# omarezz46/BayesDLL

Hardware: AMD Instinct MI355X
Metric: SG-HMC leapfrog steps/sec & HBM GB/s on ViT-L/32 params, 1/2/4/8 MI355X (higher is better)
Workload: dtype f32

## Files before the change

bayesdll_amd/_lib.py:

```python
from __future__ import annotations

import ctypes as C
import os
import threading

import torch

HERE = os.path.dirname(os.path.abspath(__file__))
LIB_PATH = os.environ.get("BDL_SGMCMC_LIB", os.path.join(HERE, "libbdl_sgmcmc.so"))

BDL_OK = 0
CSGHMC, SGHMC, SGLD, SGHMC_GRAD, SGLD_GRAD, ADAM_SGHMC, ADAM_SGHMC_GRAD = range(7)
NOISE_NONE, NOISE_BUFFER, NOISE_PHILOX = 0, 1, 2
COLLECT_NONE, COLLECT_WELFORD_INIT, COLLECT_WELFORD, COLLECT_MEAN_INIT, COLLECT_MEAN = range(5)
MIX_BARE, MIX_PIPELINED, MIX_PACED = 0, 1, 2
ATTR_HEAD, ATTR_PRIOR, ATTR_SKIP, ATTR_GUNALIGNED = 0x1, 0x2, 0x4, 0x8
FLAG_FIRST_STEP, FLAG_RECIP_DIV, FLAG_MOMENTUM, FLAG_GRAD_READY = 0x1, 0x2, 0x4, 0x8
VAR_GIVEN, VAR_RAW_MOMENTS, VAR_WELFORD = 0, 1, 2
ABI_VERSION = 8

_fp = C.c_void_p


class Segment(C.Structure):
# ... 229 lines not shown
LOWP_UNROLLS = (1, 2, 4)

LOWP_EXPORTS = {
    "bdl_lowp_step": (C.c_int, [C.POINTER(LowpArgs), C.c_void_p]),
    "bdl_lowp_shadow": (C.c_int, [C.c_void_p, C.c_void_p, C.c_void_p, C.c_int32, C.c_int64,
                                  C.c_void_p]),
}


class LayerSegment(C.Structure):
    _fields_ = [("offset", C.c_int64), ("numel", C.c_int64)]


class DiagLayersArgs(C.Structure):
    _fields_ = [("mom1", _fp), ("mom2", _fp), ("segments", _fp), ("table", _fp),
                ("workspace", _fp), ("n", C.c_int64), ("chain_groups", C.c_uint64),
                ("nsegments", C.c_int32), ("chains", C.c_int32), ("var_mode", C.c_int32),
                ("grid_blocks", C.c_int32), ("ratio", C.c_float), ("inv_ratio", C.c_float),
                ("var_floor", C.c_float), ("c1", C.c_float), ("thresholds", C.c_float * 3),
                ("pad0", C.c_int32)]


class EssLayersArgs(C.Structure):
    _fields_ = [("sM2", _fp), ("bM2", _fp), ("segments", _fp), ("table", _fp),
                ("workspace", _fp), ("n", C.c_int64), ("chain_groups", C.c_uint64),
                ("samples", C.c_int64), ("batches", C.c_int64), ("nsegments", C.c_int32),
                ("chains", C.c_int32), ("grid_blocks", C.c_int32), ("thresholds", C.c_float * 3)]


LAYERS_MAX_SEGMENTS, LAYERS_MAX_GRID = 65536, 1024

LAYERS_EXPORTS = {
    "bdl_layers_workspace_bytes": (C.c_int64, [C.c_int32, C.c_int32]),
    "bdl_chain_diag_layers": (C.c_int, [C.POINTER(DiagLayersArgs), C.c_void_p]),
    "bdl_chain_ess_layers": (C.c_int, [C.POINTER(EssLayersArgs), C.c_void_p]),
}

PREDICT_MAX_CLASSES, PREDICT_WAVE_CLASSES, PREDICT_MAX_BINS = 8192, 256, 64
PREDICT_MAX_GROUPS, PREDICT_MAX_GRID = 65535, 1024
PREDICT_RESET = 0x1


class PredictTotals(C.Structure):
    _fields_ = [("n", C.c_int64), ("n_labelled", C.c_int64), ("n_nonfinite", C.c_int64),
                ("n_wrong", C.c_int64), ("disagree_sum", C.c_int64), ("nll_sum", C.c_double),
                ("entropy_sum", C.c_double), ("expected_entropy_sum", C.c_double),
                ("mi_sum", C.c_double), ("mi_sum_wrong", C.c_double),
                ("bin_count", C.c_int64 * PREDICT_MAX_BINS),
                ("bin_hits", C.c_int64 * PREDICT_MAX_BINS),
                ("bin_conf", C.c_double * PREDICT_MAX_BINS)]


class PredictArgs(C.Structure):
    _fields_ = [("logits", _fp), ("labels", _fp), ("logp", _fp), ("entropy", _fp),
                ("expected_entropy", _fp), ("mutual_info", _fp), ("confidence", _fp),
                ("nll", _fp), ("pred", _fp), ("disagree", _fp), ("totals", _fp),
                ("workspace", _fp), ("batch", C.c_int64), ("members", C.c_int32),
                ("groups", C.c_int32), ("classes", C.c_int32), ("num_bins", C.c_int32),
                ("grid_blocks", C.c_int32), ("flags", C.c_int32),
                ("edges", C.c_float * PREDICT_MAX_BINS)]


PREDICT_EXPORTS = {
    "bdl_predict_workspace_bytes": (C.c_int64, [C.c_int32, C.c_int32]),
    "bdl_predict": (C.c_int, [C.POINTER(PredictArgs), C.c_void_p]),
}


class FnFoldArgs(C.Structure):
    _fields_ = [("logits", _fp), ("bsum", _fp), ("smean", _fp), ("sM2", _fp), ("bM2", _fp),
                ("probs", _fp), ("probe", C.c_int64), ("chain_groups", C.c_uint64),
                ("sample", C.c_int64), ("batch", C.c_int64), ("chains", C.c_int32),
                ("classes", C.c_int32), ("flags", C.c_int32), ("fs", C.c_float),
                ("fb", C.c_float), ("c", C.c_float), ("grid_blocks", C.c_int32),
                ("pad0", C.c_int32)]


FN_MAX_CLASSES, FN_WAVE_CLASSES, FN_MAX_GRID = 8192, 256, 2048

FN_EXPORTS = {
    "bdl_fn_fold": (C.c_int, [C.POINTER(FnFoldArgs), C.c_void_p]),
}

_lib = None
_lock = threading.Lock()


def lib():
    global _lib
    if _lib is not None:
        return _lib
    with _lock:
        if _lib is None:
            if not os.path.exists(LIB_PATH):
                raise RuntimeError(
                    f"bayesdll_amd: HIP library not found at {LIB_PATH}; build it with "
                    "`make -C bayesdll_amd/csrc` (or __graft_entry__.build()). There is no CPU "
                    "fallback for the fused SG-MCMC step.")
            h = C.CDLL(LIB_PATH)
            for name, (res, argt) in (list(EXPORTS.items()) + list(DIAG_EXPORTS.items())
                                      + list(CLIP_EXPORTS.items())
                                      + list(CHAIN_STEP_EXPORTS.items())
                                      + list(STATS_EXPORTS.items())
                                      + list(ESS_EXPORTS.items())
                                      + list(LOWP_EXPORTS.items())
                                      + list(LAYERS_EXPORTS.items())
                                      + list(PREDICT_EXPORTS.items())
                                      + list(FN_EXPORTS.items())):
                fn = getattr(h, name)
                fn.restype = res
                fn.argtypes = argt
            if h.bdl_version() != ABI_VERSION:
                raise RuntimeError(f"bayesdll_amd: ABI version mismatch ({h.bdl_version()} != "
                                   f"{ABI_VERSION}); rebuild the library")
            _lib = h
    return _lib


def check(rc: int, what: str):
    if rc != BDL_OK:
        msg = lib().bdl_last_error().decode(errors="replace")
        raise RuntimeError(f"{what} failed (status {rc}): {msg}")
    return rc


def ptr(t):
    return None if t is None else C.c_void_p(t.data_ptr())


def current_stream_handle(device=None):
    return C.c_void_p(torch.cuda.current_stream(device).cuda_stream)


def require_hip(t: torch.Tensor, what: str):
    if not t.is_cuda:
        raise RuntimeError(f"bayesdll_amd: {what} must live on a HIP device (got {t.device}); "
                           "the fused SG-MCMC step has no CPU path")
    if t.dtype != torch.float32:
        raise RuntimeError(f"bayesdll_amd: {what} must be float32 (got {t.dtype})")
```

bayesdll_amd/csrc/bdl_api.hip:

```cpp
#include <algorithm>
#include "bdl_chain_common.hpp"
#include "bdl_measure.h"

#include <mutex>
#include <vector>

namespace bdl {
namespace {

thread_local std::string g_last_error;

int g_blocks_per_cu = 2;
int g_unroll = 1;
int g_grid_stride = 1;

int device_cu_count() {
  static int cached[64] = {0};
  int dev = 0;
  if (hipGetDevice(&dev) != hipSuccess || dev < 0 || dev >= 64) return 256;
  if (cached[dev] == 0) {
    int cus = 0;
    if (hipDeviceGetAttribute(&cus, hipDeviceAttributeMultiprocessorCount, dev) != hipSuccess ||
        cus <= 0)
      cus = 256;
    cached[dev] = cus;
  }
  return cached[dev];
}

constexpr int kMaxNormPartials = 2048;

template <int NOISE, bool RECIP, bool PRIOR>
__device__ __forceinline__ double sqnorm_fast(const KArgs& a, const StepConst& c, int64_t gb,
                                              float ns, double acc, const float* gp) {
  constexpr int U = 2;
  f4v th[U], g[U], t0[U], ep[U];
  const f4v z = {0.f, 0.f, 0.f, 0.f};
#pragma unroll
  for (int u = 0; u < U; ++u) {
    const int64_t e = (gb + (int64_t)u * kBlock + threadIdx.x) * 4;
    t0[u] = ep[u] = z;
    th[u] = vload(a.theta + e);
    g[u] = vload(gp + e);
    if constexpr (PRIOR) t0[u] = vload(a.prior_mean + e);
    if constexpr (NOISE == BDL_NOISE_BUFFER) ep[u] = vload(a.noise + e);
  }
#pragma unroll
  for (int u = 0; u < U; ++u) {
    const int64_t gi = gb + (int64_t)u * kBlock + threadIdx.x;
    if constexpr (NOISE == BDL_NOISE_PHILOX) ep[u] = step_noise4(a, gi);
#pragma unroll
    for (int j = 0; j < 4; ++j) {
      float xt = th[u][j], xg = g[u][j], xv = 0.f;
      update_core<BDL_SGLD_GRAD, NOISE, RECIP, PRIOR, false>(a, c, 0.f, ns, xt, xg, xv, t0[u][j],
                                                             ep[u][j]);
      acc = fma((double)xg, (double)xg, acc);
    }
  }
  return acc;
}

template <int NOISE, bool RECIP>
__device__ __forceinline__ void sqnorm_body(const KArgs& a, double* __restrict__ partials) {
  __shared__ double s_wave[kBlock / 64];
  constexpr int64_t kIter = (int64_t)kBlock * 2;
  StepConst c;
  c.sgd_mom = c.sgd_mom_read = c.has_m2 = c.grad_ready = c.clip = false;
  c.inv_s2 = a.inv_s2;
  c.inv_nd = a.inv_nd;
  c.inv_ca = c.inv_cb = c.clip_coef = 1.0f;
  const int64_t ngroups = (a.n + 3) >> 2, nfull = a.n >> 2;
  stage_runs(a);
  double acc = 0.0;
  int r = find_run_lds(a.nruns, (int64_t)blockIdx.x * kIter * 4);
  for (int64_t gb = (int64_t)blockIdx.x * kIter; gb < ngroups; gb += (int64_t)gridDim.x * kIter) {
    while (r < a.nruns - 1 && run_end(r) <= gb * 4) ++r;
    const int64_t gend = min(gb + kIter, ngroups);
    const uint32_t attr = run_attr(r);
    if (gend == gb + kIter && gend <= nfull && run_end(r) >= gend * 4 && !(attr & kNoFastPath)) {
      const float ns = (attr & BDL_ATTR_HEAD) ? a.ns1 : a.ns0;
      if (attr & BDL_ATTR_PRIOR)
        acc = sqnorm_fast<NOISE, RECIP, true>(a, c, gb, ns, acc, run_grad(a, r));
      else
        acc = sqnorm_fast<NOISE, RECIP, false>(a, c, gb, ns, acc, run_grad(a, r));
    } else {
// ... 654 lines not shown
      !p.kernelParams[0]) {
    (void)hipGetLastError();
    return fail(BDL_ERR_ARG, "bdl_graph_node_step_args: not a kernel node with arguments");
  }
  {
    std::lock_guard<std::mutex> lk(g_captured_mu);
    if (std::find(g_captured_funcs.begin(), g_captured_funcs.end(), (const void*)p.func) ==
        g_captured_funcs.end())
      return fail(BDL_ERR_ARG, "bdl_graph_node_step_args: the node runs no captured step kernel");
  }
  const KArgs* ka = (const KArgs*)p.kernelParams[0];
  const int64_t v[10] = {(int64_t)(uintptr_t)ka->theta, (int64_t)(uintptr_t)ka->grad,
                         (int64_t)(uintptr_t)ka->mom,   (int64_t)(uintptr_t)ka->runs,
                         (int64_t)(uintptr_t)ka->gbase, (int64_t)ka->nruns,
                         ka->n,                          (int64_t)ka->flags,
                         (int64_t)(uintptr_t)ka->mom1,  (int64_t)(uintptr_t)ka->mom2};
  for (int i = 0; i < 10; ++i) out[i] = v[i];
  return BDL_OK;
}

int bdl_graph_redirect(void* graph_exec, void* node) {
  if (graph_exec && !node) return fail(BDL_ERR_NULL, "bdl_graph_redirect: null node");
  g_redirect_exec = (hipGraphExec_t)graph_exec;
  g_redirect_node = graph_exec ? (hipGraphNode_t)node : nullptr;
  return BDL_OK;
}

const char* bdl_last_error(void) { return g_last_error.c_str(); }

int bdl_set_launch_config(int32_t blocks_per_cu, int32_t unroll, int32_t grid_stride) {
  const int prev = (g_grid_stride << 24) | (g_blocks_per_cu << 8) | g_unroll;
  g_blocks_per_cu = blocks_per_cu > 0 ? blocks_per_cu : 2;
  g_unroll = (unroll == 1 || unroll == 2 || unroll == 4) ? unroll : 1;
  g_grid_stride = grid_stride > 0 ? 1 : 0;
  return prev;
}

int bdl_build_runs(const bdl_segment* segs, int32_t nseg, int64_t n, bdl_run* out, int32_t max_runs) {
  if (!out || (nseg > 0 && !segs)) return fail(BDL_ERR_NULL, "bdl_build_runs: null pointer");
  if (n < 0 || nseg < 0 || max_runs < 1) return fail(BDL_ERR_ARG, "bdl_build_runs: bad sizes");
  int nr = 0;
  int64_t pos = 0;
  auto push = [&](int64_t end, uint32_t attr) -> bool {
    if (end <= pos) return true;
    if (nr > 0 && out[nr - 1].attr == attr) {
      out[nr - 1].end = end;
    } else {
      if (nr >= max_runs) return false;
      out[nr].end = end;
      out[nr].attr = attr;
      out[nr].pad = 0;
      ++nr;
    }
    pos = end;
    return true;
  };
  for (int i = 0; i < nseg; ++i) {
    const bdl_segment& s = segs[i];
    if (s.offset < pos || s.numel < 0 || s.offset + s.numel > n)
      return fail(BDL_ERR_RUNS, "bdl_build_runs: segments overlap, are unsorted or exceed n");
    if (!push(s.offset, BDL_ATTR_SKIP)) return fail(BDL_ERR_ARG, "bdl_build_runs: too many runs");
    if (!push(s.offset + s.numel, s.attr & 0xFu))
      return fail(BDL_ERR_ARG, "bdl_build_runs: too many runs");
  }
  if (!push(n, BDL_ATTR_SKIP)) return fail(BDL_ERR_ARG, "bdl_build_runs: too many runs");
  if (nr == 0) {
    out[0].end = 0;
    out[0].attr = BDL_ATTR_SKIP;
    out[0].pad = 0;
    nr = 1;
  }
  return nr;
}

int bdl_sgmcmc_step(const bdl_step_args* s, void* stream) {
  return launch_step(s, nullptr, (hipStream_t)stream);
}

int bdl_sgmcmc_step_bare(const bdl_step_args* s, void* stream) {
  if (const int rc = no_redirect("bdl_sgmcmc_step_bare")) return rc;
  if (s && s->method != BDL_CSGHMC)
    return fail(BDL_ERR_ARG, "bdl_sgmcmc_step_bare: the bare sweep exists for cSGHMC only");
  return launch_step(s, nullptr, (hipStream_t)stream, true);
}

int64_t bdl_clip_workspace_bytes(int64_t n) {
  (void)n;
  return (int64_t)16 + (int64_t)kMaxNormPartials * (int64_t)sizeof(double);
}

int bdl_sgld_step_clipped(const bdl_step_args* s, float max_norm, void* workspace, void* stream) {
  if (const int rc = no_redirect("bdl_sgld_step_clipped")) return rc;
  if (!s) return fail(BDL_ERR_NULL, "bdl_sgld_step_clipped: null args");
  if (!workspace) return fail(BDL_ERR_NULL, "bdl_sgld_step_clipped: null workspace");
  if (misaligned(workspace, 15)) return fail(BDL_ERR_ALIGN, "bdl_sgld_step_clipped: workspace not 16-B aligned");
  if (s->method != BDL_SGLD)
    return fail(BDL_ERR_ARG, "bdl_sgld_step_clipped: only the SGLD sampler clips its gradient");
  if (s->flags & BDL_FLAG_GRAD_READY)
    return fail(BDL_ERR_ARG, "bdl_sgld_step_clipped: GRAD_READY is incompatible with clipping");
  if (!(max_norm > 0.0f)) return fail(BDL_ERR_ARG, "bdl_sgld_step_clipped: max_norm must be > 0");
  if (s->n < 0) return fail(BDL_ERR_ARG, "bdl_sgmcmc_step: n < 0");
  if (s->n == 0) return BDL_OK;
  if (s->noise_mode < BDL_NOISE_NONE || s->noise_mode > BDL_NOISE_PHILOX)
    return fail(BDL_ERR_ARG, "bdl_sgld_step_clipped: unknown noise mode");
  if (!s->theta || !s->prior_mean)
    return fail(BDL_ERR_NULL, "bdl_sgld_step_clipped: theta and prior_mean are required");
  if (const int rc = check_runs_and_grad(s, "bdl_sgld_step_clipped")) return rc;
  if (s->noise_mode == BDL_NOISE_BUFFER && !s->noise)
    return fail(BDL_ERR_NULL, "bdl_sgld_step_clipped: noise buffer is required");
  hipStream_t st = (hipStream_t)stream;
  float* ws = (float*)workspace;
  double* partials = reinterpret_cast<double*>(reinterpret_cast<char*>(workspace) + 16);

  KArgs a{};
  a.theta = s->theta;
  a.grad = s->grad;
  a.prior_mean = s->prior_mean;
  a.noise = s->noise;
  a.runs = s->runs;
  a.gbase = s->grad_base;
  a.nruns = s->nruns;
  a.flags = s->flags;
  a.n = s->n;
  a.goff = s->philox_offset;
  a.cgroups = (uint32_t)s->chain_groups;
  a.ns0 = s->noise_scale[0];
  a.ns1 = s->noise_scale[1];
  a.sigma2 = s->sigma2;
  a.n_data = s->n_data;
  a.seed = s->seed;
  a.chain = s->chain;
  a.step = s->step;
  a.inv_s2 = recip_or(s->inv_sigma2, s->sigma2);
  a.inv_nd = recip_or(s->inv_n_data, s->n_data);
  const int64_t ngroups = (s->n + 3) / 4;
  const int64_t iters = (ngroups + 2 * kBlock - 1) / (2 * kBlock);
  const int64_t cap = std::min<int64_t>((int64_t)device_cu_count() * g_blocks_per_cu, kMaxNormPartials);
  const int grid = (int)capped_grid(iters, cap);
  const size_t shmem = run_lds_bytes(s);
  switch (s->noise_mode) {
    case BDL_NOISE_NONE:
      hipLaunchKernelGGL(bdl_sqnorm_kernel<BDL_NOISE_NONE>, dim3(grid), dim3(kBlock), shmem, st, a, partials);
      break;
    case BDL_NOISE_BUFFER:
      hipLaunchKernelGGL(bdl_sqnorm_kernel<BDL_NOISE_BUFFER>, dim3(grid), dim3(kBlock), shmem, st, a, partials);
      break;
    default:
      hipLaunchKernelGGL(bdl_sqnorm_kernel<BDL_NOISE_PHILOX>, dim3(grid), dim3(kBlock), shmem, st, a, partials);
      break;
  }
  hipLaunchKernelGGL(bdl_clip_finalize_kernel, dim3(1), dim3(kBlock), 0, st, partials, grid, max_norm, ws);
  if (const int rc = launched("bdl_sgld_step_clipped")) return rc;
  return launch_step(s, ws, st);
}

int bdl_adam_step(const bdl_step_args* s, const bdl_adam_args* ad, void* stream) {
  if (const int rc = no_redirect("bdl_adam_step")) return rc;
  if (!s || !ad) return fail(BDL_ERR_NULL, "bdl_adam_step: null args");
  if (s->method != BDL_ADAM_SGHMC && s->method != BDL_ADAM_SGHMC_GRAD)
    return fail(BDL_ERR_ARG, "bdl_adam_step: method must be BDL_ADAM_SGHMC or BDL_ADAM_SGHMC_GRAD");
  if (s->noise_mode < BDL_NOISE_NONE || s->noise_mode > BDL_NOISE_PHILOX)
    return fail(BDL_ERR_ARG, "bdl_adam_step: unknown noise mode");
  if (s->collect < BDL_COLLECT_NONE || s->collect > BDL_COLLECT_MEAN)
    return fail(BDL_ERR_ARG, "bdl_adam_step: unknown collect mode");
  if (s->n < 0) return fail(BDL_ERR_ARG, "bdl_adam_step: n < 0");
  if (s->n == 0) return BDL_OK;
// ... 189 lines not shown
```

bayesdll_amd/flat.py:

```python
from __future__ import annotations

import contextlib
import ctypes as C

import numpy as np
import torch

from . import _lib as L
from .arena import default_grad_arena


def segment_attrs(names, readout_name, bias, requires_grad):
    attrs = []
    for nm, rg in zip(names, requires_grad):
        a = 0
        if readout_name is not None and readout_name in nm:
            a |= L.ATTR_HEAD
        if not ("bias" in nm and bias == "uninformative"):
            a |= L.ATTR_PRIOR
        if not rg:
            a |= L.ATTR_SKIP
        attrs.append(a)
    return attrs


def build_runs(offsets, numels, attrs, n):
    nseg = len(offsets)
    segs = (L.Segment * max(nseg, 1))()
    for i, (o, k, a) in enumerate(zip(offsets, numels, attrs)):
        segs[i].offset, segs[i].numel, segs[i].attr, segs[i].pad = int(o), int(k), int(a), 0
    cap = 2 * nseg + 2
    runs = (L.Run * cap)()
    nr = L.lib().bdl_build_runs(segs, nseg, int(n), runs, cap)
    if nr < 0:
        L.check(nr, "bdl_build_runs")
    out = torch.empty(nr, 2, dtype=torch.int64)
    for i in range(nr):
        out[i, 0] = runs[i].end
        out[i, 1] = runs[i].attr
    return out


GRAD_MODES = ("tensor", "flat")
MAX_TENSOR_RUNS = 2730
GRAD_TABLE_CACHE = 8


def default_grad_mode():
    import os
    m = os.environ.get("BDL_GRAD_MODE", "tensor")
    if m not in GRAD_MODES:
        raise ValueError(f"BDL_GRAD_MODE must be one of {GRAD_MODES}, got {m!r}")
    return m


COMPUTE_DTYPES = {None: None, "fp32": None, "float32": None, torch.float32: None,
                  "bf16": torch.bfloat16, "bfloat16": torch.bfloat16,
                  torch.bfloat16: torch.bfloat16}


def check_compute_dtype(compute_dtype):
    try:
        return COMPUTE_DTYPES[compute_dtype]
    except (KeyError, TypeError):
        raise ValueError(f"bayesdll_amd: compute_dtype must be fp32 or bf16, got "
                         f"{compute_dtype!r}") from None


def refuse_lowp_network(net, ntensors, grad_mode=None):
    if (grad_mode or default_grad_mode()) != "tensor":
        raise ValueError("bayesdll_amd: bf16 compute reads autograd's bf16 gradients in place: "
                         "the flat gradient vector (BDL_GRAD_MODE=flat) is not supported")
    if ntensors > MAX_TENSOR_RUNS:
        raise ValueError(f"bayesdll_amd: bf16 compute needs one run per tensor in the kernel's "
                         f"LDS table ({ntensors} parameter tensors > {MAX_TENSOR_RUNS}); the "
                         "flat gradient fallback is not supported")
    if default_grad_arena():
        raise ValueError("bayesdll_amd: bf16 compute does not support the gradient arena "
                         "(BDL_GRAD_ARENA=1)")
    fbuf = [nm for nm, b in net.named_buffers() if b.is_floating_point()]
    if fbuf:
        raise ValueError("bayesdll_amd: bf16 compute does not support networks with "
                         f"floating-point buffers (e.g. BatchNorm running statistics): {fbuf[:3]}")


class FlatState:

    def __init__(self, net, net0=None, *, readout_name=None, bias="informative",
                 need_prior=False, need_mom=True, need_noise=False, extra=(), grad_mode=None,
                 compute_dtype=None):
        named = list(net.named_parameters())
        if not named:
            raise ValueError("bayesdll_amd: the network has no parameters")
        self.compute_dtype = check_compute_dtype(compute_dtype)
        if self.compute_dtype is not None:
            refuse_lowp_network(net, len(named), grad_mode)
        self.names = [nm for nm, _ in named]
        self.params = [p for _, p in named]
        self.shapes = [tuple(p.shape) for p in self.params]
        self.numels = [p.numel() for p in self.params]
        self.offsets = np.concatenate([[0], np.cumsum(self.numels)[:-1]]).astype(np.int64).tolist()
        self.n = int(sum(self.numels))
        dev = self.params[0].device
        for nm, p in named:
            L.require_hip(p.data, f"parameter {nm!r}")
            if p.device != dev:
                raise RuntimeError("bayesdll_amd: all parameters must be on one device")
        self.device = dev
        self.readout_name = readout_name if readout_name is not None else getattr(
            net, "readout_name", None)
        self.bias = bias
        self.requires_grad = [p.requires_grad for p in self.params]
        self.grad_mode = grad_mode or default_grad_mode()
        if self.grad_mode not in GRAD_MODES:
            raise ValueError(f"grad_mode must be one of {GRAD_MODES}")
        if self.grad_mode == "tensor" and len(self.params) > MAX_TENSOR_RUNS:
            import warnings
            warnings.warn(f"bayesdll_amd: {len(self.params)} parameter tensors > "
                          f"{MAX_TENSOR_RUNS}: using the flat gradient vector")
            self.grad_mode = "flat"

        names_ = ["theta"] + (["grad"] if self.grad_mode == "flat" else []) + \
            (["mom"] if need_mom else []) + (["prior"] if need_prior else []) + list(extra)
        vecs = {nm: torch.zeros(self.n, dtype=torch.float32, device=dev) for nm in names_}
        self.extra = {nm: vecs[nm] for nm in extra}
        self.theta = vecs["theta"]
        with torch.no_grad():
            for p, o, k in zip(self.params, self.offsets, self.numels):
                self.theta[o:o + k].copy_(p.data.reshape(-1))
                p.data = self.theta[o:o + k].view(p.shape)
        self.shadow = None
        if self.compute_dtype is not None:
            self.shadow = torch.empty(self.n, dtype=self.compute_dtype, device=dev)
            self.refresh_shadow()
            for p, o, k in zip(self.params, self.offsets, self.numels):
                p.data = self.shadow[o:o + k].view(p.shape)
        self.grad = vecs["grad"].zero_() if self.grad_mode == "flat" else None
        self.gbase = None
        self._bind_grads()
        self.arena = None
        if self.grad_mode == "tensor" and default_grad_arena():
            from .arena import GradArena
            self.arena = GradArena(dev, 4 * self.n)

        self.mom = vecs["mom"].zero_() if need_mom else None
        self.prior = None
        if need_prior:
            self.prior = vecs["prior"].zero_()
            if net0 is not None:
                p0 = list(net0.parameters())
                if [tuple(q.shape) for q in p0] != self.shapes:
                    raise ValueError("bayesdll_amd: net0 does not match net's parameter shapes")
                with torch.no_grad():
                    for q, o, k in zip(p0, self.offsets, self.numels):
                        self.prior[o:o + k].copy_(q.detach().reshape(-1))
        self.noise = torch.empty(self.n, dtype=torch.float32, device=dev) if need_noise else None
        self.nonfinite = torch.zeros(1, dtype=torch.int32, device=dev)

        attrs = segment_attrs(self.names, self.readout_name, bias, self.requires_grad)
        self.attrs = attrs
        self.runs = build_runs(self.offsets, self.numels, attrs, self.n).to(dev)
        self.nruns = int(self.runs.shape[0])
        self._base_runs = (self.runs, self.nruns)
        self._skip_tables = {}
        self._grad_tables = {}
        self._untouched = ()
        self._touched = [False] * len(self.params) if self.grad_mode == "flat" else []
        self._hooks = [p.register_post_accumulate_grad_hook(self._mark(i))
                       for i, p in enumerate(self.params) if p.requires_grad] \
            if self.grad_mode == "flat" else []

    def _mark(self, i):
        touched = self._touched

        def hook(_p):
            touched[i] = True
        return hook

    @classmethod
    def from_segments(cls, segments, readout_name, *, bias="informative", device="cuda",
                      need_prior=False, need_mom=True, need_noise=False, init=None, extra=()):
        self = cls.__new__(cls)
        self.names = [nm for nm, _ in segments]
        self.shapes = [tuple(s) for _, s in segments]
        self.numels = [int(np.prod(s)) for s in self.shapes]
        self.offsets = np.concatenate([[0], np.cumsum(self.numels)[:-1]]).astype(np.int64).tolist()
        self.n = int(sum(self.numels))
        self.device = torch.device(device)
        if self.device.type == "cuda" and self.device.index is None:
            self.device = torch.device("cuda", torch.cuda.current_device())
        self.readout_name = readout_name
        self.bias = bias
        self.requires_grad = [True] * len(self.names)
        self.params = []
        self._grad_ptrs = []
        f32 = dict(dtype=torch.float32, device=self.device)
        names_ = (["theta"] if init is None else []) + ["grad"] + (["mom"] if need_mom else []) \
            + (["prior"] if need_prior else []) + list(extra)
        vecs = {nm: torch.zeros(self.n, **f32) for nm in names_}
        self.extra = {nm: vecs[nm] for nm in extra}
        self.theta = vecs["theta"] if init is None else init
        self.grad_mode = "flat"
        self.compute_dtype = None
        self.shadow = None
        self.gbase = None
        self.arena = None
        self._grad_tables = {}
        self._untouched = ()
        self.grad = vecs["grad"].zero_()
        self.mom = vecs["mom"].zero_() if need_mom else None
        self.prior = vecs["prior"].zero_() if need_prior else None
        self.noise = torch.empty(self.n, **f32) if need_noise else None
        self.nonfinite = torch.zeros(1, dtype=torch.int32, device=self.device)
        self.attrs = segment_attrs(self.names, readout_name, bias, self.requires_grad)
        self.runs = build_runs(self.offsets, self.numels, self.attrs, self.n).to(self.device)
        self.nruns = int(self.runs.shape[0])
        self._base_runs = (self.runs, self.nruns)
        self._skip_tables = {}
        self._touched = []
        self._hooks = []
        return self

    def _bind_grads(self):
        if self.grad_mode == "tensor":
            for p in self.params:
                p.grad = None
            self._grad_ptrs = [0 if rg else None for rg in self.requires_grad]
            return
        self._grad_ptrs = []
        for p, o, k, rg in zip(self.params, self.offsets, self.numels,
                               [p.requires_grad for p in self.params]):
            if rg:
                p.grad = self.grad[o:o + k].view(p.shape)
                self._grad_ptrs.append(p.grad.data_ptr())
            else:
                self._grad_ptrs.append(None)

    def zero_grad(self):
        if self.grad_mode == "tensor":
            for p in self.params:
                p.grad = None
            return
        self.grad.zero_()
        for i in range(len(self._touched)):
            self._touched[i] = False
        for p, ptr in zip(self.params, self._grad_ptrs):
            if ptr is not None and (p.grad is None or p.grad.data_ptr() != ptr):
                self._bind_grads()
                break

    def backward_routing(self):
        if self.arena is None:
            return contextlib.nullcontext()
        return self.arena.routing()

    def sync_grads(self):
        if self.grad_mode == "tensor":
            self._sync_tensor_grads()
            return
        rebind = False
        untouched = []
        for i, (p, o, k, ptr) in enumerate(zip(self.params, self.offsets, self.numels,
                                               self._grad_ptrs)):
            if ptr is None:
                continue
            g = p.grad
            if g is None:
                self.grad[o:o + k].zero_()
                untouched.append(i)
                rebind = True
            else:
                if g.data_ptr() != ptr:
                    self.grad[o:o + k].copy_(g.reshape(-1))
                    rebind = True
                if self._touched and not self._touched[i]:
                    untouched.append(i)
        if rebind:
            self._bind_grads()
        self._select_runs(tuple(untouched))

    def _select_runs(self, untouched):
        if not untouched:
            self.runs, self.nruns = self._base_runs
            return
        tab = self._skip_tables.get(untouched)
        if tab is None:
            attrs = list(self.attrs)
            for i in untouched:
                attrs[i] |= L.ATTR_SKIP
            runs = build_runs(self.offsets, self.numels, attrs, self.n).to(self.device)
            tab = self._skip_tables[untouched] = (runs, int(runs.shape[0]))
        self.runs, self.nruns = tab

    def use_tensor_grads(self, grads):
        if len(grads) != len(self.numels):
            raise ValueError("use_tensor_grads: one gradient (or None) per segment")
        self.grad_mode, self.grad = "tensor", None
        ptrs, untouched = [], []
# ... 204 lines not shown
```

bayesdll_amd/kernels.py:

```python
from __future__ import annotations

import ctypes as C
import os

import numpy as np
import torch

from . import _lib as L
from . import ess as E

DIV_MODE = os.environ.get("BDL_DIV_MODE", "recip")


def _div_flag(div_mode=None):
    return L.FLAG_RECIP_DIV if (div_mode or DIV_MODE) == "recip" else 0


def _inv(s):
    s = float(s)
    return 1.0 / s if s != 0.0 else 0.0


def _step_args(state, method, *, lrs, noise_scale, noise_mode, one_minus_alpha=1.0,
               prior_sig=0.0, sigma2=1.0, n_data=1.0, mu=0.0, first_step=False,
# ... 119 lines not shown
        _tune_kind(state, fn, kind, written)
    _use_geometry(state, kind)
    t = getattr(state, "timer", None)
    e0 = t.begin() if t is not None else None
    fn()
    if e0 is not None:
        t.end(e0, alg_bytes_per_elem(a, adam) * int(a.n))


def _written(state, method, *, grad_only, mom, extra=(), mom1=None, mom2=None):
    if grad_only:
        if getattr(state, "grad", None) is None:
            return None
        out = [state.grad]
    else:
        out = [state.theta]
    out += [t for t in (mom,) + tuple(extra) + (mom1, mom2) if t is not None]
    return out


LOWP_UNROLL = 4


def lowp_args(state, method, *, blocks=0, unroll=LOWP_UNROLL, **kw):
    if method not in (L.CSGHMC, L.SGHMC, L.SGLD):
        raise ValueError("bayesdll_amd: compute_dtype=bf16 covers the cSGHMC, SGHMC and SGLD "
                         "steps; the *_GRAD contract (the caller steps) and Adam have no bf16 form")
    if kw.get("grad_ready"):
        raise ValueError("bayesdll_amd: the bf16 step has no GRAD_READY form (no clipped step)")
    if kw.get("mom_buf") is not None:
        raise ValueError("bayesdll_amd: the bf16 step takes its SGD buffer from state.mom")
    s = _step_args(state, method, **kw)
    a = L.LowpArgs()
    for f in ("theta", "grad", "mom", "prior_mean", "noise", "mom1", "mom2", "runs", "grad_base",
              "nonfinite", "n", "nruns", "method", "noise_mode", "collect", "flags",
              "one_minus_alpha", "prior_sig", "sigma2", "n_data", "mu", "collect_a", "collect_b",
              "inv_sigma2", "inv_n_data", "inv_collect_a", "inv_collect_b", "seed", "chain",
              "step", "philox_offset", "chain_groups"):
        setattr(a, f, getattr(s, f))
    for i in range(2):
        a.lr[i], a.noise_scale[i] = s.lr[i], s.noise_scale[i]
    a.shadow = state.shadow.data_ptr()
    a.blocks, a.unroll = int(blocks), int(unroll)
    return a


def lowp_step(state, method, **kw):
    a = lowp_args(state, method, **kw)
    t = getattr(state, "timer", None)
    e0 = t.begin() if t is not None else None
    L.check(L.lib().bdl_lowp_step(a, L.current_stream_handle(state.device)), "bdl_lowp_step")
    if e0 is not None:
        s = _step_args(state, method, **{k: v for k, v in kw.items()
                                         if k not in ("blocks", "unroll")})
        t.end(e0, alg_bytes_per_elem(s) * int(a.n))


def lowp_shadow(theta, shadow):
    if shadow.dtype != torch.bfloat16 or shadow.numel() != theta.numel():
        raise ValueError("lowp_shadow: shadow must be a bf16 tensor of theta's length")
    L.require_hip(theta, "theta")
    L.check(L.lib().bdl_lowp_shadow(theta.data_ptr(), shadow.data_ptr(), None, 0,
                                    int(theta.numel()), L.current_stream_handle(theta.device)),
            "bdl_lowp_shadow")


def sgmcmc_step(state, method, **kw):
    if getattr(state, "shadow", None) is not None:
        return lowp_step(state, method, **kw)
    a = _step_args(state, method, **kw)
    mb = kw.get("mom_buf")
    wr = _written(state, method, grad_only=method in (L.SGHMC_GRAD, L.SGLD_GRAD),
                  mom=state.mom if mb is None else mb,
                  mom1=kw.get("mom1") if kw.get("collect", L.COLLECT_NONE) else None,
                  mom2=kw.get("mom2") if kw.get("collect", L.COLLECT_NONE) else None)
    _launch(state, lambda: L.check(L.lib().bdl_sgmcmc_step(a, L.current_stream_handle(state.device)),
                                   "bdl_sgmcmc_step"), a, written=wr)


def sgmcmc_step_bare(state, **kw):
    a = _step_args(state, L.CSGHMC, **kw)
    L.check(L.lib().bdl_sgmcmc_step_bare(a, L.current_stream_handle(state.device)),
            "bdl_sgmcmc_step_bare")


def adam_step(state, method, *, adam_m, adam_v, sgd_buf=None, beta1, beta2, eps, t,
              momentum_decay, nd, temperature=1.0, grad_is_mom=False, lrs, noise_mode,
              sigma2, n_data, mu=0.0, first_step=False, momentum=False, collect=L.COLLECT_NONE,
              mom1=None, mom2=None, collect_a=1.0, collect_b=1.0, seed=0, chain=0, step=0,
              div_mode=None, noise=None, philox_offset=0):
    a = _step_args(state, method, lrs=lrs, noise_scale=(0.0, 0.0), noise_mode=noise_mode,
                   one_minus_alpha=1 - momentum_decay, sigma2=sigma2, n_data=n_data, mu=mu,
                   first_step=first_step, momentum=momentum, collect=collect, mom1=mom1,
                   mom2=mom2, collect_a=collect_a, collect_b=collect_b, seed=seed, chain=chain,
                   step=step, div_mode=div_mode, noise=noise, philox_offset=philox_offset)
    ad = L.AdamArgs()
    ad.adam_m = adam_m.data_ptr()
    ad.adam_v = adam_v.data_ptr()
    ad.sgd_buf = None if sgd_buf is None else sgd_buf.data_ptr()
    ad.beta1, ad.one_minus_beta1 = float(beta1), 1 - float(beta1)
    ad.beta2, ad.one_minus_beta2 = float(beta2), 1 - float(beta2)
    bc1, bc2 = 1 - float(beta1) ** int(t), 1 - float(beta2) ** int(t)
    ad.bias_corr1, ad.bias_corr2 = bc1, bc2
    ad.eps = float(eps)
    ad.two_alpha = 2 * float(momentum_decay)
    ad.nd = float(nd)
    ad.temperature = float(temperature)
    ad.inv_bias_corr1, ad.inv_bias_corr2 = _inv(bc1), _inv(bc2)
    ad.inv_temperature = _inv(temperature)
    ad.grad_is_mom = 1 if grad_is_mom else 0
    wr = _written(state, method, grad_only=method == L.ADAM_SGHMC_GRAD, mom=state.mom,
                  extra=(adam_m, adam_v) + ((sgd_buf,) if sgd_buf is not None else ()),
                  mom1=mom1 if collect != L.COLLECT_NONE else None,
                  mom2=mom2 if collect != L.COLLECT_NONE else None)
    _launch(state, lambda: L.check(L.lib().bdl_adam_step(a, ad, L.current_stream_handle(state.device)),
                                   "bdl_adam_step"), a, ad, written=wr)


def stream_mix(reads, writes, blocks_per_cu=1, unroll=4, schedule=L.MIX_BARE):
    n = reads[0].numel()
    dev = reads[0].device
    rp = (C.c_void_p * len(reads))(*[t.data_ptr() for t in reads])
    wp = (C.c_void_p * len(writes))(*[t.data_ptr() for t in writes])
    L.check(L.lib().bdl_stream_mix_schedule(rp, len(reads), wp, len(writes), int(n),
                                            int(blocks_per_cu), int(unroll), int(schedule),
                                            L.current_stream_handle(dev)), "bdl_stream_mix")


def clip_workspace(state):
    ws = getattr(state, "_clip_ws", None)
    if ws is None:
        nbytes = int(L.lib().bdl_clip_workspace_bytes(int(state.n)))
        ws = torch.empty((nbytes + 3) // 4, dtype=torch.float32, device=state.device)
        state._clip_ws = ws
    return ws


def sgld_step_clipped(state, max_norm, **kw):
    a = _step_args(state, L.SGLD, **kw)
    _use_geometry(state)
    ws = clip_workspace(state)
    L.check(L.lib().bdl_sgld_step_clipped(a, float(max_norm), ws.data_ptr(),
                                          L.current_stream_handle(state.device)),
            "bdl_sgld_step_clipped")
    return ws


def moments_update(theta, mom1, mom2, collect, collect_a=1.0, collect_b=1.0, div_mode=None):
    L.require_hip(theta, "theta")
    a = L.MomentsArgs()
    a.theta, a.mom1 = theta.data_ptr(), mom1.data_ptr()
    a.mom2 = None if mom2 is None else mom2.data_ptr()
    a.n = theta.numel()
    a.collect = int(collect)
    a.flags = _div_flag(div_mode)
    a.collect_a, a.collect_b = float(collect_a), float(collect_b)
    a.inv_collect_a, a.inv_collect_b = _inv(collect_a), _inv(collect_b)
    L.check(L.lib().bdl_moments_update(a, L.current_stream_handle(theta.device)),
            "bdl_moments_update")


SAMPLE_GEOMETRIES = ((1, 4), (2, 4), (3, 4), (4, 4), (4, 1), (6, 1))
SAMPLE_TUNE_MIN = 1 << 22
_SAMPLE_GEOM = {}


# ... 647 lines not shown
    a.scalars = scalars.data_ptr()
    a.n1, a.chain_groups, a.chains = int(state.n1), int(state.chain_groups), int(state.K)
    a.method, a.noise_mode, a.collect = int(method), int(noise_mode), int(collect)
    a.flags = ((L.FLAG_FIRST_STEP if first_step else 0) | (L.FLAG_MOMENTUM if momentum else 0)
               | _div_flag(div_mode))
    a.blocks_per_chain, a.unroll = int(blocks_per_chain), int(unroll)
    a.collect_a, a.collect_b = float(collect_a), float(collect_b)
    a.inv_collect_a, a.inv_collect_b = _inv(collect_a), _inv(collect_b)
    a.seed = int(seed) & 0xFFFFFFFFFFFFFFFF
    a.chain = int(chain) & 0xFFFFFFFFFFFFFFFF
    a.step = int(step) & 0xFFFFFFFFFFFFFFFF
    return a


def chain_step(state, method, *, scalars, **kw):
    K_ = int(state.K)
    if (scalars.dtype != torch.float32 or not scalars.is_cuda or not scalars.is_contiguous()
            or scalars.numel() != K_ * 12 or scalars.device != state.theta.device):
        raise ValueError("chain_step: scalars must be a contiguous float32 [K, 12] tensor on the "
                         "state's device")
    if not kw.get("blocks_per_chain"):
        kw["blocks_per_chain"] = chain_step_blocks_per_chain(state.n1, K_, state.theta.device,
                                                             kw.get("unroll") or 1)
    a = chain_step_args(state, method, scalars=scalars, **kw)
    dev = state.theta.device
    t = getattr(state, "timer", None)
    e0 = t.begin() if t is not None else None
    L.check(L.lib().bdl_chain_step(a, L.current_stream_handle(dev)), "bdl_chain_step")
    if e0 is not None:
        t.end(e0, alg_bytes_per_elem(a) * int(a.n1) * K_)


def philox_normal(n, seed, chain, step, device="cuda"):
    out = torch.empty(n, dtype=torch.float32, device=device)
    L.check(L.lib().bdl_philox_normal(out.data_ptr(), int(n), int(seed), int(chain), int(step),
                                      L.current_stream_handle(out.device)), "bdl_philox_normal")
    return out


_ACTIVE = [None]
LIBRARY_DEFAULT = (2, 1, 1)


def set_launch_config(blocks_per_cu=0, unroll=0, grid_stride=0):
    _ACTIVE[0] = (int(blocks_per_cu), int(unroll), int(grid_stride))
    return L.lib().bdl_set_launch_config(int(blocks_per_cu), int(unroll), int(grid_stride))


def restore_launch_config(packed):
    return set_launch_config((packed >> 8) & 0xFFFF, packed & 0xFF, (packed >> 24) & 0xFF)


def _use_geometry(state, kind="step"):
    cfg = getattr(state, {"collect": "collect_cfg", "init": "init_cfg"}.get(kind, "launch_cfg"),
                  None)
    if cfg is None:
        cfg = getattr(state, "launch_cfg", None)
    if cfg is not None and cfg != _ACTIVE[0]:
        set_launch_config(*cfg)


AUTOTUNE_CANDIDATES = ((2, 1, 1), (1, 4, 1), (3, 1, 1), (2, 4, 1), (1, 2, 1), (2, 2, 1))
AUTOTUNE_BY_METHOD = {
    "csghmc": AUTOTUNE_CANDIDATES + ((3, 4, 1), (1, 1, 1)),
    "sgld": AUTOTUNE_CANDIDATES + ((3, 4, 1), (4, 4, 1), (1, 1, 1)),
    "adam": AUTOTUNE_CANDIDATES + ((1, 1, 1), (4, 4, 1)),
}
_TUNED = {}
_TUNED_COLLECT = {}
COLLECT_EXTRA = ((1, 1, 1),)


ADAM_EXTRA = ("adam_m", "adam_v", "sgd_buf")


def _scratch_launcher(n, dev, method):
    return _scratch_launchers(n, dev, method)[0]


def _scratch_launchers(n, dev, method):
    from .flat import FlatState, moment_pair
    st = FlatState.from_segments([("w", (int(n),))], None, device=dev,
                                 need_prior=method != "csghmc",
                                 extra=ADAM_EXTRA if method == "adam" else ())
    st.theta.zero_()
    if method == "csghmc":
        kw = dict(lrs=(1e-4, 1e-4), noise_scale=(0.0, 0.0), noise_mode=L.NOISE_NONE,
                  one_minus_alpha=0.9, prior_sig=1.0)

        def launch():
            sgmcmc_step(st, L.CSGHMC, **kw)
    elif method == "sgld":
        st.prior.zero_()
        kw = dict(lrs=(1e-4, 1e-4), noise_scale=(1e-3, 1e-3), noise_mode=L.NOISE_PHILOX,
                  sigma2=1.0, n_data=1e6, mu=0.5, momentum=True)

        def launch():
            sgmcmc_step(st, L.SGLD, **kw)
    elif method == "adam":
        st.prior.zero_()
        m, v, buf = (st.extra[k] for k in ADAM_EXTRA)
        kw = dict(adam_m=m, adam_v=v, sgd_buf=buf, beta1=0.9, beta2=0.999, eps=1e-8, t=3,
                  momentum_decay=0.1, nd=0.01, lrs=(1e-4, 1e-4), noise_mode=L.NOISE_PHILOX,
                  sigma2=1.0, n_data=1e6, mu=0.5, momentum=True)

        def launch():
            adam_step(st, L.ADAM_SGHMC, **kw)
    else:
        raise ValueError(f"unknown method {method!r}")
    moms = []

    def launch_collect():
        if not moms:
            moms.extend(moment_pair(int(n), dev) if method == "csghmc" else
                        (torch.zeros_like(st.theta), torch.zeros_like(st.theta)))
            moms[0].copy_(st.theta)
            moms[1].zero_()
        if method == "csghmc":
            sgmcmc_step(st, L.CSGHMC, lrs=(1e-4, 1e-4), noise_scale=(1e-7, 1e-7),
                        noise_mode=L.NOISE_PHILOX, one_minus_alpha=0.9, prior_sig=1.0,
                        collect=L.COLLECT_WELFORD, mom1=moms[0], mom2=moms[1], collect_a=3.0)
        elif method == "sgld":
            sgmcmc_step(st, L.SGLD, collect=L.COLLECT_MEAN, mom1=moms[0], mom2=moms[1],
                        collect_a=2.0, collect_b=3.0, **kw)
        else:
            adam_step(st, L.ADAM_SGHMC, collect=L.COLLECT_MEAN, mom1=moms[0], mom2=moms[1],
                      collect_a=2.0, collect_b=3.0, **kw)
    return launch, launch_collect


def _device(device):
    return torch.device(device) if device is not None else torch.device(
        "cuda", torch.cuda.current_device())


def autotune(n, device=None, reps=6, candidates=None, method="csghmc", collect=False):
    import numpy as np
    dev = _device(device)
    if candidates is None:
        candidates = AUTOTUNE_BY_METHOD.get(method, AUTOTUNE_CANDIDATES)
    launch, launch_collect = _scratch_launchers(n, dev, method)

    def pick(fn, cands):
        times = measure(fn, cands, reps)
        top = sorted(times, key=times.get)[:3]
        again = measure(fn, top, 2 * reps)
        for cfg in top:
            times[cfg] = 0.5 * (times[cfg] + again[cfg])
        return min(top, key=times.get), times

    def measure(fn, cfgs, k):
        out = {}
        for cfg in cfgs:
            set_launch_config(*cfg)
            for _ in range(2):
                fn()
            ev = [(torch.cuda.Event(enable_timing=True), torch.cuda.Event(enable_timing=True))
                  for _ in range(k)]
            for e0, e1 in ev:
                e0.record()
                fn()
                e1.record()
            torch.cuda.synchronize(dev)
            out[cfg] = float(np.median([a.elapsed_time(b) for a, b in ev]))
        return out

    best, times = pick(launch, candidates)
# ... 111 lines not shown
```

Baseline: 1002.

## Pick momentum buffer placement by timing candidate allocations at construction

```diff
diff --git a/bayesdll_amd/_lib.py b/bayesdll_amd/_lib.py
--- a/bayesdll_amd/_lib.py
+++ b/bayesdll_amd/_lib.py
@@ -335,6 +335,21 @@
     "bdl_fn_fold": (C.c_int, [C.POINTER(FnFoldArgs), C.c_void_p]),
 }
 
+PLACE_MAX_CAND = 8
+
+
+class PlaceDesc(C.Structure):
+    _fields_ = [("theta", _fp), ("grad", _fp), ("cand", C.POINTER(C.c_void_p)), ("runs", _fp),
+                ("n", C.c_int64), ("nruns", C.c_int32), ("ncand", C.c_int32), ("warm", C.c_int32),
+                ("reps", C.c_int32), ("blocks_per_cu", C.c_int32), ("unroll", C.c_int32),
+                ("tie_margin", C.c_float), ("pad", C.c_int32), ("stream", C.c_void_p)]
+
+
+PLACE_EXPORTS = {
+    "bdl_place_pick": (C.c_int, [C.POINTER(PlaceDesc), C.POINTER(C.c_int32),
+                                 C.POINTER(C.c_float)]),
+}
+
 _lib = None
 _lock = threading.Lock()
 
@@ -363,6 +378,11 @@
                 fn = getattr(h, name)
                 fn.restype = res
                 fn.argtypes = argt
+            for name, (res, argt) in PLACE_EXPORTS.items():
+                fn = getattr(h, name, None)
+                if fn is not None:
+                    fn.restype = res
+                    fn.argtypes = argt
             if h.bdl_version() != ABI_VERSION:
                 raise RuntimeError(f"bayesdll_amd: ABI version mismatch ({h.bdl_version()} != "
                                    f"{ABI_VERSION}); rebuild the library")
diff --git a/bayesdll_amd/csrc/bdl_api.hip b/bayesdll_amd/csrc/bdl_api.hip
--- a/bayesdll_amd/csrc/bdl_api.hip
+++ b/bayesdll_amd/csrc/bdl_api.hip
@@ -1,6 +1,7 @@
 #include <algorithm>
 #include "bdl_chain_common.hpp"
 #include "bdl_measure.h"
+#include "bdl_place.h"
 
 #include <mutex>
 #include <vector>
@@ -821,6 +822,96 @@
   if (s && s->method != BDL_CSGHMC)
     return fail(BDL_ERR_ARG, "bdl_sgmcmc_step_bare: the bare sweep exists for cSGHMC only");
   return launch_step(s, nullptr, (hipStream_t)stream, true);
+}
+
+int bdl_place_pick(const bdl_place_desc* d, int32_t* best, float* ms) {
+  const char* const W = "bdl_place_pick";
+  if (const int rc = no_redirect(W)) return rc;
+  if (!d || !best || !ms) return fail(BDL_ERR_ARG, std::string(W) + ": null descriptor or output");
+  if (!d->theta || !d->grad || !d->cand || !d->runs)
+    return fail(BDL_ERR_ARG, std::string(W) + ": theta, grad, cand and runs are required");
+  if (d->n <= 0) return fail(BDL_ERR_ARG, std::string(W) + ": n must be positive");
+  if (d->ncand < 1 || d->ncand > BDL_PLACE_MAX_CAND)
+    return fail(BDL_ERR_ARG, std::string(W) + ": ncand must be 1 .. 8");
+  if (d->reps < 1 || d->warm < 0)
+    return fail(BDL_ERR_ARG, std::string(W) + ": reps >= 1 and warm >= 0 are required");
+  if (!(d->tie_margin >= 0.f))
+    return fail(BDL_ERR_ARG, std::string(W) + ": tie_margin must be >= 0");
+  if (d->blocks_per_cu < 0 || d->unroll < 0 ||
+      (d->unroll != 0 && d->unroll != 1 && d->unroll != 2 && d->unroll != 4))
+    return fail(BDL_ERR_ARG, std::string(W) + ": geometry is 0 (installed) or blocks_per_cu > 0, "
+                "unroll 1 / 2 / 4");
+  const uintptr_t bytes = (uintptr_t)d->n * sizeof(float);
+  auto overlaps = [bytes](const void* a, const void* b) {
+    const uintptr_t x = (uintptr_t)a, y = (uintptr_t)b;
+    return x < y + bytes && y < x + bytes;
+  };
+  for (int i = 0; i < d->ncand; ++i) {
+    if (!d->cand[i]) return fail(BDL_ERR_ARG, std::string(W) + ": null candidate");
+    if (overlaps(d->cand[i], d->theta) || overlaps(d->cand[i], d->grad))
+      return fail(BDL_ERR_ARG, std::string(W) + ": a candidate overlaps theta or grad");
+    if (misaligned(d->cand[i], 15))
+      return fail(BDL_ERR_ALIGN, std::string(W) + ": candidate not 16-B aligned");
+  }
+  hipStream_t stream = (hipStream_t)d->stream;
+  hipStreamCaptureStatus cs = hipStreamCaptureStatusNone;
+  if (hipStreamIsCapturing(stream, &cs) != hipSuccess) (void)hipGetLastError();
+  if (cs != hipStreamCaptureStatusNone)
+    return fail(BDL_ERR_ARG, std::string(W) + ": the stream is capturing");
+
+  bdl_step_args s{};
+  s.theta = d->theta;
+  s.grad = const_cast<float*>(d->grad);
+  s.runs = d->runs;
+  s.nruns = d->nruns;
+  s.method = BDL_CSGHMC;
+  s.noise_mode = BDL_NOISE_NONE;
+  s.collect = BDL_COLLECT_NONE;
+  s.n = d->n;
+  s.one_minus_alpha = s.sigma2 = s.n_data = s.collect_a = s.collect_b = 1.f;
+
+  hipEvent_t e0 = nullptr, e1 = nullptr;
+  if (hipEventCreate(&e0) != hipSuccess || hipEventCreate(&e1) != hipSuccess) {
+    if (e0) (void)hipEventDestroy(e0);
+    (void)hipGetLastError();
+    return fail(BDL_ERR_LAUNCH, std::string(W) + ": hipEventCreate failed");
+  }
+  const int pb = g_blocks_per_cu, pu = g_unroll, pg = g_grid_stride;
+  if (d->blocks_per_cu > 0) g_blocks_per_cu = d->blocks_per_cu;
+  if (d->unroll > 0) g_unroll = d->unroll;
+  g_grid_stride = 1;
+  int rc = BDL_OK;
+  for (int i = 0; i < d->ncand && rc == BDL_OK; ++i) {
+    s.mom = d->cand[i];
+    for (int k = 0; k < d->warm && rc == BDL_OK; ++k) rc = launch_step(&s, nullptr, stream, true);
+    if (rc != BDL_OK) break;
+    hipError_t err = hipEventRecord(e0, stream);
+    for (int k = 0; k < d->reps && rc == BDL_OK; ++k) rc = launch_step(&s, nullptr, stream, true);
+    if (rc != BDL_OK) break;
+    float t = 0.f;
+    if (err == hipSuccess) err = hipEventRecord(e1, stream);
+    if (err == hipSuccess) err = hipEventSynchronize(e1);
+    if (err == hipSuccess) err = hipEventElapsedTime(&t, e0, e1);
+    if (err != hipSuccess) {
+      (void)hipGetLastError();
+      rc = fail(BDL_ERR_LAUNCH, std::string(W) + ": timing failed: " + hipGetErrorString(err));
+      break;
+    }
+    ms[i] = t / (float)d->reps;
+  }
+  g_blocks_per_cu = pb;
+  g_unroll = pu;
+  g_grid_stride = pg;
+  (void)hipEventDestroy(e0);
+  (void)hipEventDestroy(e1);
+  if (rc != BDL_OK) return rc;
+  float lo = ms[0];
+  for (int i = 1; i < d->ncand; ++i) lo = std::min(lo, ms[i]);
+  const float bound = lo * (1.f + d->tie_margin);
+  int b = 0;
+  while (b < d->ncand - 1 && !(ms[b] <= bound)) ++b;
+  *best = b;
+  return BDL_OK;
 }
 
 int64_t bdl_clip_workspace_bytes(int64_t n) {
diff --git a/bayesdll_amd/flat.py b/bayesdll_amd/flat.py
--- a/bayesdll_amd/flat.py
+++ b/bayesdll_amd/flat.py
@@ -84,11 +84,58 @@
                          f"floating-point buffers (e.g. BatchNorm running statistics): {fbuf[:3]}")
 
 
+PLACE_MIN_BYTES = 256 << 20
+PLACE_NCAND = 4
+
+
+def place_enabled():
+    import os
+    return os.environ.get("BDL_PLACE_MOM", "1") != "0"
+
+
+def place_wanted(n, device, place_min_bytes=PLACE_MIN_BYTES, ncand=PLACE_NCAND):
+    if not place_enabled() or 4 * n <= place_min_bytes or ncand < 2 or device.type != "cuda":
+        return False
+    from . import kernels as K
+    return K.place_available()
+
+
+def alloc_momentum(theta, grad, runs_host, *, place_min_bytes=PLACE_MIN_BYTES,
+                   ncand=PLACE_NCAND):
+    n, dev = theta.numel(), theta.device
+    f32 = dict(dtype=torch.float32, device=dev)
+    if not place_wanted(n, dev, place_min_bytes, ncand):
+        return torch.zeros(n, **f32), None
+    from . import kernels as K
+    ncand = min(int(ncand), L.PLACE_MAX_CAND)
+    cands = [torch.empty(n, **f32) for _ in range(ncand)]
+    g = grad if grad is not None else torch.empty(n, **f32)
+    runs = runs_host.to(dev)
+    best, ms = K.place_pick(theta, g, cands, runs, int(runs.shape[0]))
+    mom = cands[best]
+    del cands, g, runs
+    return mom.zero_(), {"chosen": best, "ms": [round(t, 4) for t in ms], "ncand": ncand,
+                         "geometry": K.PLACE_GEOMETRY, "warm": K.PLACE_WARM,
+                         "reps": K.PLACE_REPS, "tie_margin": K.PLACE_TIE_MARGIN}
+
+
 class FlatState:
+
+    def _alloc_vectors(self, names_, runs_host, place_min_bytes, theta=None):
+        f32 = dict(dtype=torch.float32, device=self.device)
+        vecs, self.placement = {}, None
+        for nm in names_:
+            if nm == "mom":
+                vecs[nm], self.placement = alloc_momentum(
+                    vecs["theta"] if theta is None else theta, vecs.get("grad"), runs_host,
+                    place_min_bytes=place_min_bytes)
+            else:
+                vecs[nm] = torch.zeros(self.n, **f32)
+        return vecs
 
     def __init__(self, net, net0=None, *, readout_name=None, bias="informative",
                  need_prior=False, need_mom=True, need_noise=False, extra=(), grad_mode=None,
-                 compute_dtype=None):
+                 compute_dtype=None, place_min_bytes=PLACE_MIN_BYTES):
         named = list(net.named_parameters())
         if not named:
             raise ValueError("bayesdll_amd: the network has no parameters")
@@ -122,7 +169,9 @@
 
         names_ = ["theta"] + (["grad"] if self.grad_mode == "flat" else []) + \
             (["mom"] if need_mom else []) + (["prior"] if need_prior else []) + list(extra)
-        vecs = {nm: torch.zeros(self.n, dtype=torch.float32, device=dev) for nm in names_}
+        attrs = segment_attrs(self.names, self.readout_name, bias, self.requires_grad)
+        runs_host = build_runs(self.offsets, self.numels, attrs, self.n)
+        vecs = self._alloc_vectors(names_, runs_host, place_min_bytes)
         self.extra = {nm: vecs[nm] for nm in extra}
         self.theta = vecs["theta"]
         with torch.no_grad():
@@ -157,9 +206,8 @@
         self.noise = torch.empty(self.n, dtype=torch.float32, device=dev) if need_noise else None
         self.nonfinite = torch.zeros(1, dtype=torch.int32, device=dev)
 
-        attrs = segment_attrs(self.names, self.readout_name, bias, self.requires_grad)
         self.attrs = attrs
-        self.runs = build_runs(self.offsets, self.numels, attrs, self.n).to(dev)
+        self.runs = runs_host.to(dev)
         self.nruns = int(self.runs.shape[0])
         self._base_runs = (self.runs, self.nruns)
         self._skip_tables = {}
@@ -179,7 +227,8 @@
 
     @classmethod
     def from_segments(cls, segments, readout_name, *, bias="informative", device="cuda",
-                      need_prior=False, need_mom=True, need_noise=False, init=None, extra=()):
+                      need_prior=False, need_mom=True, need_noise=False, init=None, extra=(),
+                      place_min_bytes=PLACE_MIN_BYTES):
         self = cls.__new__(cls)
         self.names = [nm for nm, _ in segments]
         self.shapes = [tuple(s) for _, s in segments]
@@ -197,7 +246,9 @@
         f32 = dict(dtype=torch.float32, device=self.device)
         names_ = (["theta"] if init is None else []) + ["grad"] + (["mom"] if need_mom else []) \
             + (["prior"] if need_prior else []) + list(extra)
-        vecs = {nm: torch.zeros(self.n, **f32) for nm in names_}
+        self.attrs = segment_attrs(self.names, readout_name, bias, self.requires_grad)
+        runs_host = build_runs(self.offsets, self.numels, self.attrs, self.n)
+        vecs = self._alloc_vectors(names_, runs_host, place_min_bytes, theta=init)
         self.extra = {nm: vecs[nm] for nm in extra}
         self.theta = vecs["theta"] if init is None else init
         self.grad_mode = "flat"
@@ -212,8 +263,7 @@
         self.prior = vecs["prior"].zero_() if need_prior else None
         self.noise = torch.empty(self.n, **f32) if need_noise else None
         self.nonfinite = torch.zeros(1, dtype=torch.int32, device=self.device)
-        self.attrs = segment_attrs(self.names, readout_name, bias, self.requires_grad)
-        self.runs = build_runs(self.offsets, self.numels, self.attrs, self.n).to(self.device)
+        self.runs = runs_host.to(self.device)
         self.nruns = int(self.runs.shape[0])
         self._base_runs = (self.runs, self.nruns)
         self._skip_tables = {}
diff --git a/bayesdll_amd/kernels.py b/bayesdll_amd/kernels.py
--- a/bayesdll_amd/kernels.py
+++ b/bayesdll_amd/kernels.py
@@ -225,6 +225,35 @@
     a = _step_args(state, L.CSGHMC, **kw)
     L.check(L.lib().bdl_sgmcmc_step_bare(a, L.current_stream_handle(state.device)),
             "bdl_sgmcmc_step_bare")
+
+
+PLACE_GEOMETRY = (1, 4)
+PLACE_WARM, PLACE_REPS = 4, 8
+PLACE_TIE_MARGIN = 0.03
+
+
+def place_available():
+    try:
+        return hasattr(L.lib(), "bdl_place_pick")
+    except (RuntimeError, OSError):
+        return False
+
+
+def place_pick(theta, grad, cands, runs, nruns, *, warm=PLACE_WARM, reps=PLACE_REPS,
+               geometry=PLACE_GEOMETRY, tie_margin=PLACE_TIE_MARGIN):
+    d = L.PlaceDesc()
+    d.theta, d.grad, d.runs = theta.data_ptr(), grad.data_ptr(), runs.data_ptr()
+    ptrs = (C.c_void_p * max(len(cands), 1))(*[c.data_ptr() for c in cands])
+    d.cand = ptrs
+    d.n, d.nruns, d.ncand = int(theta.numel()), int(nruns), len(cands)
+    d.warm, d.reps = int(warm), int(reps)
+    d.blocks_per_cu, d.unroll = int(geometry[0]), int(geometry[1])
+    d.tie_margin = float(tie_margin)
+    d.stream = torch.cuda.current_stream(theta.device).cuda_stream
+    best = C.c_int32(-1)
+    ms = (C.c_float * max(len(cands), 1))()
+    L.check(L.lib().bdl_place_pick(d, C.byref(best), ms), "bdl_place_pick")
+    return int(best.value), [float(x) for x in ms[:len(cands)]]
 
 
 def adam_step(state, method, *, adam_m, adam_v, sgd_buf=None, beta1, beta2, eps, t,
@@ -1038,7 +1067,8 @@
     from .flat import FlatState, moment_pair
     st = FlatState.from_segments([("w", (int(n),))], None, device=dev,
                                  need_prior=method != "csghmc",
-                                 extra=ADAM_EXTRA if method == "adam" else ())
+                                 extra=ADAM_EXTRA if method == "adam" else (),
+                                 place_min_bytes=1 << 62)
     st.theta.zero_()
     if method == "csghmc":
         kw = dict(lrs=(1e-4, 1e-4), noise_scale=(0.0, 0.0), noise_mode=L.NOISE_NONE,
diff --git a/include/bdl_place.h b/include/bdl_place.h
--- /dev/null
+++ b/include/bdl_place.h
@@ -0,0 +1,37 @@
+#ifndef BDL_PLACE_H
+#define BDL_PLACE_H
+
+#include <stdint.h>
+
+#include "bdl_sgmcmc.h"
+
+#ifdef __cplusplus
+extern "C" {
+#endif
+
+#define BDL_PLACE_MAX_CAND 8
+
+typedef struct bdl_place_desc {
+  float* theta;
+  const float* grad;
+  float* const* cand;
+  const bdl_run* runs;
+  int64_t n;
+  int32_t nruns;
+  int32_t ncand;
+  int32_t warm;
+  int32_t reps;
+  int32_t blocks_per_cu;
+  int32_t unroll;
+  float tie_margin;
+  int32_t pad;
+  void* stream;
+} bdl_place_desc;
+
+int bdl_place_pick(const bdl_place_desc* d, int32_t* best, float* ms );
+
+#ifdef __cplusplus
+}
+#endif
+
+#endif
```

New measurement: 954.0. -4.8%, worse.
